# sdfgeoff/stereo_depth_estimation

Measured on AMD Instinct MI355X. Metric: stereo pairs/s training @320x240 bf16, 1/2/4/8 MI355X; EPE vs ref, higher is better.
Workload: dtype bf16

## Files before the change

stereo_depth_estimation_amd/csrc/conv_halo.hip:

```cpp
#include "common.h"
#include "halo_util.h"

namespace {

constexpr int CK = 32;
#ifndef WG_EXP
#define WG_EXP 0
#endif
typedef float f32x16 __attribute__((ext_vector_type(16)));

struct HaloSrc {
    const __bf16* p0;
    const __bf16* p1;
    const float *sc0, *sh0, *sc1, *sh1;
    int c0, c1, x0, x1;
    int ctot;
};
static inline HaloSrc make_halo_src(const sd_src& s) {
    HaloSrc h;
    h.p0 = (const __bf16*)s.ptr[0];
    h.p1 = (const __bf16*)s.ptr[1];
    h.sc0 = s.scale[0];
    h.sh0 = s.shift[0];
    h.sc1 = s.scale[1];
    h.sh1 = s.shift[1];
    h.c0 = s.chans[0];
    h.c1 = s.chans[1];
    h.x0 = s.xform[0];
    h.x1 = s.xform[1];
    h.ctot = s.chans[0] + s.chans[1];
    return h;
}

__device__ __forceinline__ uint4 bnrelu8(uint4 raw, const float* sc, const float* sh) {
    float v[8];
    const unsigned w[4] = {raw.x, raw.y, raw.z, raw.w};
#pragma unroll
    for (int i = 0; i < 4; ++i) {
        v[2 * i] = __uint_as_float(w[i] << 16);
        v[2 * i + 1] = __uint_as_float(w[i] & 0xffff0000u);
    }
    xform8(v, sc, sh, 0);
// ... 86 lines not shown
    int th, tw, tiles_x;
    int tiles, nsp;
    int nblk, gper;
    int hw, nhalo;
    const __bf16* wp;
    int N, kpad;
    int wsplit;
    const float* osc;
    const float* osh;
    int epi;
    __bf16* out0;
    __bf16* out1;
    int n_split;
    float* stats;
    int xcd;
    int prio;
    unsigned long long* dbg;
    const __bf16* by;
    const float *bsc, *bsh, *bmu, *bis;
    int ksplit, gblk, cps;
    int npix;
    float* part;
};

#ifndef HC_ST_AUX
#define HC_ST_AUX 2
#endif
#ifndef HC_WDMA
#define HC_WDMA 1
#endif
#ifndef HC_VR
#define HC_VR 1
#endif
__device__ __forceinline__ void stats_add(float* own, const uint4 v, const bool live) {
    const unsigned wv[4] = {live ? v.x : 0u, live ? v.y : 0u, live ? v.z : 0u, live ? v.w : 0u};
#pragma unroll
    for (int q = 0; q < 4; ++q) {
        const f32x2 x = {__uint_as_float(wv[q] << 16), __uint_as_float(wv[q] & 0xffff0000u)};
        f32x2 sm = {own[4 * q], own[4 * q + 1]}, sq = {own[4 * q + 2], own[4 * q + 3]};
        sm += x;
        sq = __builtin_elementwise_fma(x, x, sq);
        own[4 * q] = sm.x;
        own[4 * q + 1] = sm.y;
        own[4 * q + 2] = sq.x;
        own[4 * q + 3] = sq.y;
    }
}
template <bool B> struct BoolC { static constexpr bool v = B; };
constexpr int PERSIST_BLOCKS = 256;
constexpr int SBN_MAX = 1024;
constexpr int HMAX = 384;
__host__ __device__ constexpr int halo_px_cap(int RT, int CK) { return RT == 4 ? 640 : (RT == 3 && CK == 16 ? 512 : 384); }
__host__ __device__ constexpr int halo_ld(int CK) { return CK == 8 ? 8 : CK + 8; }
__host__ __device__ constexpr int wrow_ld(int CK) { return CK == 8 ? 88 : 9 * CK + 8; }
__device__ __forceinline__ int wswz(int row) { return ((row >> 2) & 1) * 2; }

template <int PPX>
__device__ __forceinline__ int ld_pixel(int item) { return (item / (8 * PPX)) * 8 + (item & 7); }
template <int PPX>
__device__ __forceinline__ int ld_piece(int item) { return (item >> 3) % PPX; }

template <int NT, int RT, int CK, bool STATS, bool WCONST, int IT, bool BNS, bool OAFF, bool RAW>
__device__ __forceinline__ void halo_conv_body(const HFwdArgs& p) {
    static_assert(!(OAFF && (STATS || BNS)), "the affine epilogue stores eval-mode outputs (no statistics)");
    constexpr int BN = 32 * NT;
    constexpr int PPX = CK / 8;
    constexpr bool M16 = CK == 32 && IT == 1 && !BNS;
    constexpr int HX_LD = halo_ld(CK), W_LD = M16 ? 9 * CK : wrow_ld(CK);
    constexpr int HPX = IT == 2 ? 384 : halo_px_cap(RT, CK);
    constexpr int HP = (HPX * PPX + 255) / 256;
    constexpr int WPIECES = BN * 9 * PPX;
    constexpr int W_PER_THREAD = (WPIECES + 255) / 256;
    static_assert(!M16 || (HP * 256 == HPX * PPX && HPX % 16 == 0), "M16: the loader pieces tile the halo exactly");
    constexpr int HALO_ITEM = M16 ? HPX * CK : HP * 256 / PPX * HX_LD;
    constexpr int HALO_ELEMS = IT * HALO_ITEM, W_ELEMS = BN * W_LD, BUF = HALO_ELEMS + W_ELEMS;
    static_assert(IT == 1 || (IT == 2 && HP * IT <= 16), "item masks fit 16 bits");
    constexpr int KS = (9 * CK + 15) / 16;
    __shared__ __attribute__((aligned(16))) __bf16 smem[2 * BUF];
    constexpr int SCR_PX = M16 ? 16 : 32;
    __shared__ __attribute__((aligned(16))) __bf16 scr[4 * SCR_PX * BN];

    const int tid = threadIdx.x, lane = tid & 63;
    const bool is_loader = (tid >> 6) >= 4;
    const int wid = (tid >> 6) & 3;
    const int bid = p.xcd ? (blockIdx.x & 7) * (gridDim.x >> 3) + (blockIdx.x >> 3) : blockIdx.x;
    const int ks = bid / p.gblk, bb = bid - ks * p.gblk;
    const int nb = bb % p.nblk, slot = bb / p.nblk;
    const int n0 = nb * BN;
    const int nc0 = (p.a.c0 + CK - 1) / CK;
    const int ncp = nc0 + (p.a.c1 + CK - 1) / CK;
    const int nch_v = p.wsplit ? 2 * ncp : ncp;
    const int c_lo = ks * p.cps;
    const int nchunks = (c_lo + p.cps < nch_v ? c_lo + p.cps : nch_v) - c_lo;
    const int wct = p.wsplit ? 2 * p.a.ctot : p.a.ctot;
    const int mvalid = p.th * p.tw;
    const int my_items = slot < p.nsp ? (p.nsp - 1 - slot) / p.gper + 1 : 0;
    const int total = (my_items + IT - 1) / IT * nchunks;
#ifndef HC_LS_N32
#define HC_LS_N32 2
#endif
    constexpr int LS = NT == 1 && CK == 8 ? 4 : (NT == 1 && CK == 32 ? HC_LS_N32 : 2);
    const int padded = (total + LS - 1) / LS * LS;

    __shared__ __attribute__((aligned(16))) float sbn[2 * SBN_MAX + 2 * CK];
    __shared__ __attribute__((aligned(16))) float oaff[OAFF ? 2 * BN : 4];
    auto fill_tables = [&]() __attribute__((always_inline)) {
        if constexpr (OAFF) {
            for (int c = tid; c < 2 * BN; c += 512) {
                const int ch = n0 + (c < BN ? c : c - BN);
                oaff[c] = ch < p.N ? (c < BN ? p.osc : p.osh)[ch] : 0.f;
            }
        }
        for (int c = tid; c < p.a.ctot; c += 512) {
            const bool first = c < p.a.c0;
            const int cl = first ? c : c - p.a.c0;
            const bool bn = (first ? p.a.x0 : p.a.x1) == SD_BNRELU;
            sbn[c] = bn ? (first ? p.a.sc0 : p.a.sc1)[cl] : 1.f;
            sbn[SBN_MAX + c] = bn ? (first ? p.a.sh0 : p.a.sh1)[cl] : 0.f;
        }
    };
    float* const redf = sbn;
    static_assert(4 * BN * 2 <= 2 * SBN_MAX, "redf fits in sbn");

    if (p.prio != 0 && (__builtin_amdgcn_readfirstlane(threadIdx.x) >= 256) == (p.prio == 2))
        __builtin_amdgcn_s_setprio(1);
    if (is_loader) {
        const int ltid = wid * 64 + lane;
        constexpr unsigned OOB = 0x80000000u;
        const int hw_img = p.H * p.W;
        const int lpiece = ld_piece<PPX>(ltid);
        unsigned pgeo[HP];
#pragma unroll
        for (int i = 0; i < HP; ++i) {
            const int px = ld_pixel<PPX>(ltid + i * 256);
            const int hy = px / p.hw;
            pgeo[i] = px < p.nhalo ? ((unsigned)hy << 16) | (unsigned)(px - hy * p.hw) : 0xffffffffu;
        }
        int hpx[IT][HP];
        const __bf16* ib0[IT];
        const __bf16* ib1[IT];
        int ld_pass = 0, ld_cc = 0;
        auto geometry = [&]() __attribute__((always_inline)) {
#pragma unroll
            for (int u = 0; u < IT; ++u) {
                const int itm = ld_pass * IT + u;
                const bool live = itm < my_items;
                const int sp = slot + (live ? itm : 0) * p.gper;
                const int b = sp / p.tiles, tl = sp - b * p.tiles;
                const int ty = tl / p.tiles_x;
                const int h0 = ty * p.th - 1, w0 = (tl - ty * p.tiles_x) * p.tw - 1;
                ib0[u] = p.a.p0 + (size_t)b * hw_img * p.a.c0;
                ib1[u] = p.a.c1 ? p.a.p1 + (size_t)b * hw_img * p.a.c1 : p.a.p0;
#pragma unroll
                for (int i = 0; i < HP; ++i) {
                    const int h = h0 + (int)(pgeo[i] >> 16), w = w0 + (int)(pgeo[i] & 0xffffu);
                    const bool in = live & (pgeo[i] != 0xffffffffu) & (h >= 0) & (w >= 0) & (h < p.H) & (w < p.W);
                    hpx[u][i] = in ? h * p.W + w : -1;
                }
            }
        };
        const __amdgpu_buffer_rsrc_t wrs =
            __builtin_amdgcn_make_buffer_rsrc((void*)p.wp, (short)0, p.N * p.kpad * 2, 0x00020000);
        constexpr bool WDMA = HC_WDMA && M16 && IT == 1 && (!WCONST || RAW);
        unsigned woff[W_PER_THREAD];
#pragma unroll
        for (int i = 0; i < W_PER_THREAD; ++i) {
            const int item = ltid + i * 256;
            const int co = item / (9 * PPX), r = item - co * (9 * PPX), tap = r / PPX, sp = r - tap * PPX;
// ... 60 lines not shown
        };
        auto load_w = [&]() __attribute__((always_inline)) { load_w_into(wr); };
        auto dma_w = [&](int buf) __attribute__((always_inline)) {
            const int wv = c_lo + w_cc;
            const bool lo = wv >= ncp;
            const int wc = lo ? wv - ncp : wv;
            const bool s1 = wc >= nc0;
            const int cl = (s1 ? wc - nc0 : wc) * CK;
            if (++w_cc == nchunks) w_cc = 0;
            const unsigned soff = __builtin_amdgcn_readfirstlane(((s1 ? p.a.c0 : 0) + cl + (lo ? p.a.ctot : 0)) * 2);
            const unsigned m0b = __builtin_amdgcn_readfirstlane(lds_w0 + (unsigned)(buf * BUF * 2));
#pragma unroll
            for (int j = 0; j < WDI; ++j) {
                if (NWI % 4 != 0 && wid_u * WDI + j >= NWI) break;
                unsigned keep;
                asm volatile(
                    "s_mov_b32 %0, m0\n\t"
                    "s_mov_b32 m0, %2\n\t"
                    "s_nop 0\n\t"
                    "buffer_load_dwordx4 %1, %3, %4 offen lds\n\t"
                    "s_mov_b32 m0, %0"
                    : "=&s"(keep)
                    : "v"(wdoff[j]), "s"(m0b + (unsigned)j * 1024u), "s"(wrs), "s"(soff)
                    : "memory");
            }
        };
        if constexpr (RAW) {
            static_assert(M16 && PPX == 4 && HPX % 64 == 0 && WDMA, "RAW: the M16 piece-major halo, weights by DMA");
            constexpr int HI = HPX / 64;
            unsigned hg[HI];
#pragma unroll
            for (int i = 0; i < HI; ++i) {
                const int px = i * 64 + lane;
                const int hy = px / p.hw;
                hg[i] = px < p.nhalo ? ((unsigned)hy << 16) | (unsigned)(px - hy * p.hw) : 0xffffffffu;
            }
            int hp[HI];
            const __bf16 *rb0 = p.a.p0, *rb1 = p.a.p0;
            int r_pass = 0, r_cc = 0;
            auto rgeo = [&]() __attribute__((always_inline)) {
                const bool live = r_pass < my_items;
                const int sp = slot + (live ? r_pass : 0) * p.gper;
                const int b = sp / p.tiles, tl = sp - b * p.tiles;
                const int ty = tl / p.tiles_x;
                const int h0 = ty * p.th - 1, w0 = (tl - ty * p.tiles_x) * p.tw - 1;
                rb0 = p.a.p0 + (size_t)b * hw_img * p.a.c0;
                rb1 = p.a.c1 ? p.a.p1 + (size_t)b * hw_img * p.a.c1 : p.a.p0;
#pragma unroll
                for (int i = 0; i < HI; ++i) {
                    const int h = h0 + (int)(hg[i] >> 16), w = w0 + (int)(hg[i] & 0xffffu);
                    const bool in = live & (hg[i] != 0xffffffffu) & (h >= 0) & (w >= 0) & (h < p.H) & (w < p.W);
                    hp[i] = in ? h * p.W + w : -1;
                }
            };
            rgeo();
            const unsigned lds_h0 = (unsigned)(uintptr_t)smem + (unsigned)(wid_u * HPX * 16);
            fill_tables();
            __syncthreads();
            if constexpr (WCONST) {
                dma_w(0);
                dma_w(1);
            }
            for (int g = 0; g < padded; ++g) {
                if (g < total) {
                    const int hv = c_lo + r_cc;
                    const int hc = hv >= ncp ? hv - ncp : hv;
                    const bool s1 = hc >= nc0;
// ... 94 lines not shown
#pragma unroll
            for (int u = 0; u < IT; ++u)
#pragma unroll
            for (int i = 0; i < HP; ++i) {
                const int item = ltid + i * 256;
                uint4 v = q.hr[u][i];
                const bool ok = (q.m >> (u * HP + i)) & 1u;
                if (q.bn && !(WG_EXP & 2048)) {
                    v = bnrelu_pk(v, s0, s1, h0, h1);
                    v = ok ? v : make_uint4(0, 0, 0, 0);
                }
                const int hoff = M16 ? ld_piece<PPX>(item) * HPX * 8 + ld_pixel<PPX>(item) * 8
                                     : ld_pixel<PPX>(item) * HX_LD + ld_piece<PPX>(item) * 8;
                *reinterpret_cast<uint4*>(hx + u * HALO_ITEM + hoff) = v;
            }
            if constexpr (!WCONST && !WDMA) if (!(WG_EXP & 131072)) store_w(buf);
        };
        constexpr std::integral_constant<int, 0> S0{};
        constexpr std::integral_constant<int, 1> S1{};
        constexpr std::integral_constant<int, 2> S2{};
        constexpr std::integral_constant<int, 3> S3{};
        constexpr bool DG = (WG_EXP & 1024) != 0;
        unsigned long long t_st = 0, t_ld = 0, t_br = 0, t0 = 0, t_all = DG ? __builtin_amdgcn_s_memtime() : 0;
        auto stamp = [&](unsigned long long& acc_) __attribute__((always_inline)) {
            if (DG) {
                asm volatile("s_waitcnt lgkmcnt(0)" ::: "memory");
                const unsigned long long t1 = __builtin_amdgcn_s_memtime();
                acc_ += t1 - t0;
                t0 = t1;
            } else if (WG_EXP & 8192) {
                asm volatile("s_waitcnt lgkmcnt(0)" ::: "memory");
            }
        };
        auto iter = [&](auto U) __attribute__((always_inline)) {
            if (DG) t0 = __builtin_amdgcn_s_memtime();
            if (!(WG_EXP & 65536)) store(U, decltype(U)::value & 1);
            stamp(t_st);
            if constexpr (WDMA) {
                __builtin_amdgcn_sched_barrier(0);
                dma_w(decltype(U)::value & 1);
                __builtin_amdgcn_sched_barrier(0);
            } else if constexpr (!WCONST) {
                if (!(WG_EXP & 65536)) load_w();
            }
            if (!(WG_EXP & 65536)) load(U);
            stamp(t_ld);
            if constexpr (WDMA && !(WG_EXP & 4194304)) {
                __builtin_amdgcn_sched_barrier(0);
                asm volatile("s_waitcnt vmcnt(%0)" ::"i"(IT * HP) : "memory");
            }
            __syncthreads();
            stamp(t_br);
        };
        uint4 wr2[WCONST ? W_PER_THREAD : 1];
        if (total > 0) {
            geometry();
            if constexpr (WCONST) {
                load_w();
                if (nchunks > 1) load_w_into(wr2);
                __builtin_amdgcn_sched_barrier(0);
            }
            load(S0);
            __builtin_amdgcn_sched_barrier(0);
            if constexpr (LS == 4) {
                load(S1);
                __builtin_amdgcn_sched_barrier(0);
                load(S2);
                __builtin_amdgcn_sched_barrier(0);
            }
            if constexpr (!WCONST && !WDMA) load_w();
            __builtin_amdgcn_sched_barrier(0);
            if constexpr (LS == 4) load(S3);
            else load(S1);
        }
        fill_tables();
        __syncthreads();
        if (total > 0) {
            if constexpr (WCONST) {
                store_w(0);
                if (nchunks > 1) store_w_from(1, wr2);
                else store_w(1);
            }
            for (int gi = 0; gi < total; gi += LS) {
                iter(S0);
                iter(S1);
                if constexpr (LS == 4) {
                    iter(S2);
                    iter(S3);
                }
            }
        }
        if (DG && p.dbg && lane == 0) {
            unsigned long long* d = p.dbg + ((size_t)blockIdx.x * 8 + 4 + wid) * 4;
            d[0] = t_st;
            d[1] = t_ld;
            d[2] = t_br;
            d[3] = __builtin_amdgcn_s_memtime() - t_all;
        }
        __syncthreads();
        return;
    }

    fill_tables();
    __syncthreads();
    static_assert(!(STATS && BNS), "one kind of stats rows");
    constexpr int NOWN = STATS || BNS ? 16 : 1;
    float own[NOWN];
#pragma unroll
    for (int j = 0; j < NOWN; ++j) own[j] = 0.f;
    constexpr int PPP = NT * 4;
    constexpr bool VR32 = HC_VR && !M16 && NT == 1 && RT == 4 && CK == 32 && IT == 1;
    auto tile_T = [&](int i) { return M16 || VR32 ? wid * RT + i : wid + 4 * i; };
    constexpr bool VR = HC_VR && M16 && NT == 1 && RT == 4;
    int abase[RT];
#pragma unroll
    for (int i = 0; i < RT; ++i) {
        const int m = tile_T(i) * 32 + (lane & 31);
        const int hm = m / p.tw, wm = m - hm * p.tw;
        abase[i] = m < mvalid ? hm * p.hw + wm : 0;
    }
    int abase16[M16 ? 2 * RT : 1];
    if constexpr (M16) {
#pragma unroll
        for (int i = 0; i < 2 * RT; ++i) {
            const int m = tile_T(i >> 1) * 32 + (i & 1) * 16 + (lane & 15);
            const int hm = m / p.tw, wm = m - hm * p.tw;
            abase16[i] = (lane >> 4) * HPX * 8 + (m < mvalid ? hm * p.hw + wm : 0) * 8;
        }
    }
    f32x16 acc[M16 ? 1 : IT][M16 ? 1 : RT][M16 ? 1 : NT];
    f32x4 acc4[M16 ? 2 * RT : 1][M16 ? 2 * NT : 1];
    constexpr int EPR = 64 / PPP;
    constexpr int ER = 32 / EPR;
    auto swz = [](int j, int px) { return NT == 2 ? j ^ (px & 7) : j ^ ((px >> 1) & 3); };
    unsigned erel[(RT * ER + 1) / 2];
#pragma unroll
    for (int k = 0; k < (RT * ER + 1) / 2; ++k) erel[k] = 0xffffffffu;
#pragma unroll
    for (int i = 0; i < RT; ++i)
#pragma unroll
        for (int r = 0; r < ER; ++r) {
            const int m = tile_T(i) * 32 + r * EPR + lane / PPP;
            const int hm = m / p.tw, wm = m - hm * p.tw;
            const unsigned v = m < mvalid ? (unsigned)((hm << 9) | wm) : 0xffffu;
            const int k = i * ER + r;
            erel[k / 2] = (erel[k / 2] & ~(0xffffu << (16 * (k & 1)))) | (v << (16 * (k & 1)));
        }
    constexpr bool EFAST = M16 && !(NT == 2 && RT == 3);
    constexpr int NEO = EFAST ? RT * ER : 1;
    int eoff[NEO];
#pragma unroll
    for (int k = 0; k < NEO; ++k) {
        const int m = tile_T(k / ER) * 32 + (k % ER) * EPR + lane / PPP;
        const int hm = m / p.tw, wm = m - hm * p.tw;
        eoff[k] = m < mvalid ? hm * p.W + wm : -1;
    }
    __bf16* const scw = scr + wid * SCR_PX * BN;
    constexpr int NBK = BNS ? 8 : 1, NYQ = BNS ? RT * ER : 1;
    BnsK bk[NBK / 2 > 0 ? NBK / 2 : 1];
    uint4 yq[NYQ];
    if constexpr (BNS) {
        const int c = n0 + (lane % PPP) * 8;
#pragma unroll
        for (int q = 0; q < 4; ++q) {
            float v[4][2];
#pragma unroll
            for (int h = 0; h < 2; ++h) {
                const int ch = c + 2 * q + h;
                const bool cin = ch < p.N;
                v[0][h] = cin ? p.bsc[ch] : 0.f;
                v[1][h] = cin ? p.bsh[ch] : 0.f;
                v[2][h] = cin ? p.bis[ch] : 0.f;
                v[3][h] = cin ? -p.bmu[ch] * p.bis[ch] : 0.f;
            }
            bk[q].sc = f32x2{v[0][0], v[0][1]};
            bk[q].sh = f32x2{v[1][0], v[1][1]};
            bk[q].is = f32x2{v[2][0], v[2][1]};
            bk[q].nmi = f32x2{v[3][0], v[3][1]};
        }
    }
    auto prefetch_y = [&](int itm) __attribute__((always_inline)) {
        const int sp = slot + itm * p.gper;
        const int b = sp / p.tiles, tl = sp - b * p.tiles;
        const int ty = tl / p.tiles_x;
        const int h0 = ty * p.th, w0 = (tl - ty * p.tiles_x) * p.tw;
        const int hw_img = p.H * p.W;
        const __amdgpu_buffer_rsrc_t ry = __builtin_amdgcn_make_buffer_rsrc(
            (void*)(p.by + (size_t)b * hw_img * p.N), (short)0, hw_img * p.N * 2, 0x00020000);
#pragma unroll
        for (int k = 0; k < RT * ER; ++k) {
            const unsigned rel = (erel[k / 2] >> (16 * (k & 1))) & 0xffffu;
            const int h = h0 + (int)(rel >> 9), w = w0 + (int)(rel & 511u);
            const int c = n0 + (lane % PPP) * 8;
            const bool in = (rel != 0xffffu) & (h < p.H) & (w < p.W) & (c < p.N);
            const unsigned off = in ? (unsigned)((h * p.W + w) * p.N + c) * 2u : 0x80000000u;
            const auto v = __builtin_amdgcn_raw_buffer_load_b128(ry, off, 0, 0);
            yq[k] = make_uint4(v[0], v[1], v[2], v[3]);
        }
    };

    constexpr bool DG = (WG_EXP & 1024) != 0;
    unsigned long long t_cp = 0, t_ep = 0, t_br = 0, t0 = 0, t_all = DG ? __builtin_amdgcn_s_memtime() : 0;
    int cc = 0, pass = 0;
    for (int gi = 0; gi < total; ++gi) {
        if (DG) t0 = __builtin_amdgcn_s_memtime();
        if (WG_EXP & 16384) {
            asm volatile("" ::: "memory");
            __builtin_amdgcn_sched_barrier(0);
        }
        __syncthreads();
        if (DG) {
            const unsigned long long t1 = __builtin_amdgcn_s_memtime();
            t_br += t1 - t0;
            t0 = t1;
        }
        if (WG_EXP & 16384) {
            asm volatile("" ::: "memory");
            __builtin_amdgcn_sched_barrier(0);
        }
        if (cc == 0) {
            if constexpr (M16) {
#pragma unroll
                for (int i = 0; i < 2 * RT; ++i)
#pragma unroll
                    for (int t = 0; t < 2 * NT; ++t) acc4[i][t] = f32x4{0.f, 0.f, 0.f, 0.f};
            } else {
#pragma unroll
            for (int u = 0; u < IT; ++u)
#pragma unroll
            for (int i = 0; i < RT; ++i)
#pragma unroll
                for (int t = 0; t < NT; ++t)
#pragma unroll
                    for (int r = 0; r < 16; ++r) acc[u][i][t][r] = 0.f;
            }
        }
        if constexpr (BNS) {
            if (cc == nchunks - 1) prefetch_y(pass);
        }
        const __bf16* hx = smem + (gi & 1) * BUF;
        const __bf16* wl = hx + HALO_ELEMS;
#ifndef HC_PF
#define HC_PF 1
#endif
        constexpr int PF = HC_PF;
        bf16x8 af[PF + 1][IT][RT], bfr[PF + 1][NT];
        auto read_frags = [&](int step) {
// ... 120 lines not shown
                __builtin_amdgcn_sched_barrier(0);
#pragma unroll
                for (int kh = 0; kh < 3; ++kh) {
                    const int r = hr - kh;
                    if (r < 0 || r >= R) continue;
                    acc[0][r][0] = __builtin_amdgcn_mfma_f32_32x32x16_bf16(av[kh][ch], xv[st % (PV + 1)], acc[0][r][0], 0,
                                                                           0, 0);
                }
                __builtin_amdgcn_sched_barrier(0);
            }
        } else if (!(WG_EXP & 8)) {
#pragma unroll
        for (int step = 0; step < PF; ++step) read_frags(step);
#pragma unroll
        for (int step = 0; step < KS; ++step) {
            if (step + PF < KS) read_frags(step + PF);
            __builtin_amdgcn_sched_barrier(0);
            const int sl = step % (PF + 1);
#pragma unroll
            for (int u = 0; u < IT; ++u)
#pragma unroll
            for (int i = 0; i < RT; ++i)
#pragma unroll
                for (int t = 0; t < NT; ++t)
                    acc[u][i][t] = __builtin_amdgcn_mfma_f32_32x32x16_bf16(bfr[sl][t], af[sl][u][i], acc[u][i][t], 0, 0, 0);
            __builtin_amdgcn_sched_barrier(0);
        }
        }

        if (DG) {
            const unsigned long long t1 = __builtin_amdgcn_s_memtime();
            t_cp += t1 - t0;
            t0 = t1;
        }
        if (WG_EXP & 16384) {
            asm volatile("" ::: "memory");
            __builtin_amdgcn_sched_barrier(0);
        }
        if (++cc == nchunks) {
#pragma unroll
          for (int u = 0; u < IT; ++u) {
            const int item = pass * IT + u;
            if (IT > 1 && item >= my_items) break;
            const int sp = slot + item * p.gper;
            const int b = sp / p.tiles, tl = sp - b * p.tiles;
            const int ty = tl / p.tiles_x;
            const int h0 = ty * p.th, w0 = (tl - ty * p.tiles_x) * p.tw;
            const int hw_img = p.H * p.W;
            if constexpr (!STATS && !BNS) {
                if (p.part) {
                    float* const pk = p.part + ((size_t)ks * p.npix + (size_t)b * hw_img) * p.N;
                    auto put = [&](int m, int c, float a0, float a1, float a2, float a3) __attribute__((always_inline)) {
                        const int hm = m / p.tw, wm = m - hm * p.tw;
                        if ((m < mvalid) & (h0 + hm < p.H) & (w0 + wm < p.W) & (n0 + c < p.N))
                            *reinterpret_cast<float4*>(pk + ((size_t)(h0 + hm) * p.W + w0 + wm) * p.N + n0 + c) =
                                make_float4(a0, a1, a2, a3);
                    };
                    if constexpr (M16) {
#pragma unroll
                        for (int i2 = 0; i2 < 2 * RT; ++i2)
#pragma unroll
                            for (int t = 0; t < 2 * NT; ++t)
                                put(tile_T(i2 >> 1) * 32 + (i2 & 1) * 16 + (lane & 15), t * 16 + 4 * (lane >> 4),
                                    acc4[i2][t][0], acc4[i2][t][1], acc4[i2][t][2], acc4[i2][t][3]);
                    } else {
#pragma unroll
// ... 157 lines not shown
                    const unsigned rel = (erel[(i * ER + r) / 2] >> (16 * ((i * ER + r) & 1))) & 0xffffu;
                    const int h = h0 + (int)(rel >> 9), w = w0 + (int)(rel & 511u);
                    const bool live = (rel != 0xffffu) & (h < p.H) & (w < p.W);
                    const bool in = live & !(WG_EXP & 4096);
                    const int pix = h * p.W + w, c = n0 + j * 8;
                    if constexpr (BNS) {
                        bns_add(own, v, yq[i * ER + r], live, bk);
                    }
                    if constexpr (STATS) {
                        stats_add(own, v, live);
                    }
                    __attribute__((ext_vector_type(4))) unsigned data = {v.x, v.y, v.z, v.w};
                    if (!split) {
                        const unsigned off = (in & (c < p.N)) ? (unsigned)(pix * p.N + c) * 2u : 0x80000000u;
                        __builtin_amdgcn_raw_buffer_store_b128(data, rs0, off, 0, HC_ST_AUX);
                    } else {
                        const unsigned o0 = (in & (c < ns)) ? (unsigned)(pix * ns + c) * 2u : 0x80000000u;
                        const unsigned o1 = (in & (c >= ns) & (c < p.N)) ? (unsigned)(pix * (p.N - ns) + c - ns) * 2u
                                                                       : 0x80000000u;
                        __builtin_amdgcn_raw_buffer_store_b128(data, rs0, o0, 0, HC_ST_AUX);
                        __builtin_amdgcn_raw_buffer_store_b128(data, rs1, o1, 0, HC_ST_AUX);
                    }
                }
              }
            }
            }
          }
            cc = 0;
            ++pass;
            if (DG) {
                const unsigned long long t1 = __builtin_amdgcn_s_memtime();
                t_ep += t1 - t0;
                t0 = t1;
            }
        }
    }
    for (int e = total; e < padded; ++e) __syncthreads();
    if (DG && p.dbg && lane == 0) {
        unsigned long long* d = p.dbg + ((size_t)blockIdx.x * 8 + wid) * 4;
        d[0] = t_cp;
        d[1] = t_ep;
        d[2] = t_br;
        d[3] = __builtin_amdgcn_s_memtime() - t_all;
    }

    if constexpr (STATS || BNS) {
#pragma unroll
        for (int k = 0; k < NOWN; ++k) {
#pragma unroll
            for (int o = PPP; o < 64; o <<= 1) own[k] += __shfl_xor(own[k], o);
        }
        if (lane < PPP) {
#pragma unroll
            for (int k = 0; k < NOWN; ++k)
                redf[(wid * BN + lane * 8 + k / 2) * 2 + (k & 1)] =
                    own[(k & ~3) | ((k & 1) << 1) | ((k >> 1) & 1)];
        }
    }
    __syncthreads();
    if ((STATS || BNS) && tid < BN && n0 + tid < p.N) {
        float s = 0.f, ss = 0.f;
#pragma unroll
        for (int w = 0; w < 4; ++w) {
            s += redf[(w * BN + tid) * 2];
            ss += redf[(w * BN + tid) * 2 + 1];
        }
        reinterpret_cast<float2*>(p.stats)[(size_t)slot * p.N + n0 + tid] = make_float2(s, ss);
    }
}

template <int NT, int RT, int CK, bool STATS, bool WCONST, int IT, bool BNS, bool OAFF = false, bool RAW = false>
__global__ __launch_bounds__(512) void k_halo_conv(const HFwdArgs p) {
    halo_conv_body<NT, RT, CK, STATS, WCONST, IT, BNS, OAFF, RAW>(p);
}

struct HWgArgs {
    const __bf16* dy;
    HaloSrc x;
    int H, W, th, tw, hw, nhalo, tiles_x, tiles_y, ntiles, tiles_per_split;
    int M, N;
    float* slab;
    int xcd;
    unsigned long long* dbg;
    const __bf16* bda;
    const __bf16* by;
    const float *bsc, *bsh, *bmu, *bis, *bcoef;
    int ncc;
};

constexpr int XW_LD = CK + 16;
__device__ __forceinline__ int wg_pixel(int item) { return (item >> 5) * 8 + ((item >> 3) & 1) * 4 + ((item >> 1) & 3); }
__device__ __forceinline__ int wg_piece(int item) { return (item & 1) + ((item >> 4) & 1) * 2; }
constexpr int HP_PER_THREAD = HMAX * (CK / 8) / 256;
constexpr int WG_MAXPX = 256;



template <int COUT, bool BNB, bool X8 = false>
__global__ __launch_bounds__(256, 2) void k_halo_wgrad(const HWgArgs p) {
    constexpr int DY_LD = COUT + 16;
// ... 311 lines not shown
        for (int h = 0; h < 2; ++h) {
            const int m = ks * 16 + pk + 8 * h;
            const int hm = m / p.tw;
            const int px = m < mvalid ? hm * HP + (m - hm * p.tw) : 0;
            xoff[ks][h] = (unsigned)(px * XLD + ch16) * 2u;
        }
    const unsigned aoff = (unsigned)(pk * DLD + ch16) * 2u;
    switch (__builtin_amdgcn_readfirstlane(wid)) {
    case 0: ws_mfma32_tiles<HP, DLD, XLD, DY_E, BUF, 0>(p, smem, lane, cc, mb, split, ntile, xoff, aoff); break;
    case 1: ws_mfma32_tiles<HP, DLD, XLD, DY_E, BUF, 1>(p, smem, lane, cc, mb, split, ntile, xoff, aoff); break;
    case 2: ws_mfma32_tiles<HP, DLD, XLD, DY_E, BUF, 2>(p, smem, lane, cc, mb, split, ntile, xoff, aoff); break;
    default: ws_mfma32_tiles<HP, DLD, XLD, DY_E, BUF, 3>(p, smem, lane, cc, mb, split, ntile, xoff, aoff); break;
    }
}

template <int COUT, int CIB, int HP, int HR, bool BNB, bool SPAN, bool MF32 = false>
__global__ __launch_bounds__(512, 2 * ws_blocks_per_cu(COUT, CIB)) void k_halo_wgrad_ws(const HWgArgs p) {
    constexpr int KS = WS_TPX / 32;
    constexpr int NCI = CIB / 16, NCO = 4 / NCI, RM = COUT / 16 / NCO;
    constexpr int DPP = COUT / 8, XPP = CIB / 8;
    constexpr int PAD = MF32 ? 32 : 16;
    constexpr int DLD = COUT + PAD, XLD = CIB + PAD;
    constexpr int DYP = WS_TPX * DPP / 256;
    constexpr int HXP = (HP * HR * XPP + 255) / 256;
    constexpr int DY_E = WS_TPX * DLD, BUF = DY_E + HXP * (256 / XPP) * XLD;
    static_assert(RM >= 1 && NCI * NCO == 4, "wave grid");
    static_assert(!MF32 || (COUT == 64 && CIB == 64 && !SPAN), "MF32: 64 x 64 blocks");
    static_assert(2 * BUF * 2 <= 160 * 1024, "LDS");
    __shared__ __attribute__((aligned(16))) __bf16 smem[2 * BUF];

    const int tid = threadIdx.x, lane = tid & 63;
    const bool is_loader = tid >= 256;
    const int wid = (tid >> 6) & 3;
    int cc = blockIdx.x, zb = blockIdx.z, split = blockIdx.y;
    if (p.xcd) {
        const int G = gridDim.x * gridDim.y * gridDim.z;
        const int L = blockIdx.x + gridDim.x * (blockIdx.y + gridDim.y * blockIdx.z);
        const int lg = (L & 7) * (G >> 3) + (L >> 3);
        cc = lg % gridDim.x;
        const int r = lg / gridDim.x;
        zb = r % gridDim.z;
        split = r / gridDim.z;
    }
    const int mb = zb * COUT;
    const int t_begin = split * p.tiles_per_split;
    const int ntile = max(0, min(p.ntiles, t_begin + p.tiles_per_split) - t_begin);
    const int mvalid = p.th * p.tw;

    if (is_loader) {
        constexpr int prio = (COUT == 128 && !BNB) ? 0 : WS_PRIO;
        if (prio) __builtin_amdgcn_s_setprio(prio);
        const int ltid = tid - 256;
        const int dpiece = ltid % DPP, dpix0 = ltid / DPP, xpiece = ltid % XPP, xpix0 = ltid / XPP;
        unsigned dyrc[(DYP + 1) / 2], hgeo[(HXP + 1) / 2];
#pragma unroll
        for (int i = 0; i < DYP; i += 2) {
            unsigned e[2];
#pragma unroll
            for (int h = 0; h < 2; ++h) {
                const int m = dpix0 + (256 / DPP) * (i + h);
                const int hm = m / p.tw;
                e[h] = (i + h < DYP && m < mvalid) ? (unsigned)(hm << 8 | (m - hm * p.tw)) : 0xffffu;
            }
            dyrc[i / 2] = e[0] | e[1] << 16;
        }
#pragma unroll
        for (int i = 0; i < HXP; i += 2) {
            unsigned e[2];
#pragma unroll
            for (int h = 0; h < 2; ++h) {
                const int px = xpix0 + (256 / XPP) * (i + h);
                const int hy = px / HP, hx = px - hy * HP;
                e[h] = (i + h < HXP && hy < p.th + 2 && hx < p.hw) ? (unsigned)(hy << 8 | hx) : 0xffffu;
            }
            hgeo[i / 2] = e[0] | e[1] << 16;
        }
        const HaloCol hc = halo_col(p.x, cc * CIB + xpiece * 8, p.slab);
        const bool bsrc1 = cc * CIB >= p.x.c0;
        const __bf16* xsrc = bsrc1 ? p.x.p1 : p.x.p0;
        const int xC = SPAN ? hc.C : (bsrc1 ? p.x.c1 : p.x.c0);
        const bool lsrc1 = SPAN && cc * CIB + xpiece * 8 >= p.x.c0;
        int dpo[DYP], xpo[HXP];
#pragma unroll
        for (int i = 0; i < DYP; ++i) {
            const unsigned rc = (dyrc[i / 2] >> (16 * (i & 1))) & 0xffffu;
            dpo[i] = ((int)(rc >> 8) * p.W + (int)(rc & 0xff)) * p.M + mb + dpiece * 8;
        }
#pragma unroll
        for (int i = 0; i < HXP; ++i) {
            const unsigned gg = (hgeo[i / 2] >> (16 * (i & 1))) & 0xffffu;
            xpo[i] = (((int)(gg >> 8) - 1) * p.W + (int)(gg & 0xff) - 1) * xC + hc.c;
        }
        constexpr bool DYDMA = WS_DYDMA && !BNB && !SPAN && (DLD * 2) % 16 == 0;
        constexpr int RS = DLD / 8;
        constexpr int NDI = (WS_TPX * RS + 63) / 64;
        constexpr int DDI = DYDMA ? (NDI + 3) / 4 : 1;
        const int lw = __builtin_amdgcn_readfirstlane(wid);
        int ddo[DDI];
        unsigned ddrc[DDI];
        if constexpr (DYDMA) {
#pragma unroll
            for (int j = 0; j < DDI; ++j) {
                const int k = lw * DDI + j, sl = k * 64 + lane;
                const int m = sl / RS, pc = sl - m * RS;
                const int hm = m / p.tw, wm = m - hm * p.tw;
                const bool ok = k < NDI && pc < DPP && m < mvalid && m < WS_TPX;
                ddo[j] = ok ? (hm * p.W + wm) * p.M + mb + pc * 8 : -1;
                ddrc[j] = ok ? (unsigned)(hm << 8 | wm) : 0xffffu;
            }
        }
        const unsigned lds_dy0 = (unsigned)(uintptr_t)smem + (unsigned)(lw * DDI) * 1024u;
        constexpr int NK = BNB ? 8 : 1;
        float ksc[NK], ksh[NK], kB[NK], kC[NK];
        if constexpr (BNB) {
            const int c = mb + dpiece * 8;
#pragma unroll
            for (int j = 0; j < 8; ++j) {
                const float k1 = p.bcoef[3 * (c + j) + 1], k2 = p.bcoef[3 * (c + j) + 2];
                const float is = p.bis[c + j], sc = p.bsc[c + j], sh = p.bsh[c + j];
                ksc[j] = sc;
                ksh[j] = sh;
                kB[j] = -is * k2;
                kC[j] = is * k2 * sh + sc * (p.bmu[c + j] * is * k2 - k1);
            }
        }
        constexpr int DYY = BNB ? DYP : 1;
        constexpr unsigned OOB = 0x80000000u;
        struct TSet {
            uint4 d[DYP], x[HXP];
            unsigned xm;
            uint4 y[DYY];
            int dbase;
            int img;
            bool wr;
        };
        TSet sa, sb;
        auto load = [&](TSet& q, int tile) __attribute__((always_inline)) {
            if (WG_EXP & 256) return;
// ... 86 lines not shown
                    (WG_EXP & 2048) ? q.x[i] : halo_finish_pk(hc, (q.xm >> i) & 1u, q.x[i]);
        };
        constexpr bool DG = (WG_EXP & 1024) != 0;
        unsigned long long t_st = 0, t_ld = 0, t_br = 0, t0 = 0, t1 = 0, t_all = DG ? __builtin_amdgcn_s_memtime() : 0;
        auto dma_dy = [&](int buf, int tile) __attribute__((always_inline)) {
            const int tx = tile % p.tiles_x;
            const int rest = tile / p.tiles_x;
            const int ty = rest % p.tiles_y, b = rest / p.tiles_y;
            const int h0 = ty * p.th, w0 = tx * p.tw;
            const int nimg = p.H * p.W;
            const __amdgpu_buffer_rsrc_t rdy = __builtin_amdgcn_make_buffer_rsrc(
                (void*)(p.dy + (size_t)b * nimg * p.M), (short)0, nimg * p.M * 2, 0x00020000);
            int rhi = p.H - h0, chi = p.W - w0;
            if (tile >= t_begin + ntile) rhi = 0;
            const int dbase = (h0 * p.W + w0) * p.M;
            const unsigned m0b = __builtin_amdgcn_readfirstlane(lds_dy0 + (unsigned)(buf * BUF * 2));
#pragma unroll
            for (int j = 0; j < DDI; ++j) {
                if (NDI % 4 != 0 && lw * DDI + j >= NDI) break;
                const bool ok = (ddo[j] >= 0) & ((int)(ddrc[j] >> 8) < rhi) & ((int)(ddrc[j] & 0xffu) < chi);
                const unsigned off = ok ? (unsigned)(dbase + ddo[j]) * 2u : OOB;
                unsigned keep;
                asm volatile(
                    "s_mov_b32 %0, m0\n\t"
                    "s_mov_b32 m0, %2\n\t"
                    "s_nop 0\n\t"
                    "buffer_load_dwordx4 %1, %3, 0 offen lds\n\t"
                    "s_mov_b32 m0, %0"
                    : "=&s"(keep)
                    : "v"(off), "s"(m0b + (unsigned)j * 1024u), "s"(rdy)
                    : "memory");
            }
        };
        auto iter = [&](TSet& q, int buf, int tile) __attribute__((always_inline)) {
            if (DG) t0 = __builtin_amdgcn_s_memtime();
            store(q, buf);
            if (DG) { asm volatile("s_waitcnt lgkmcnt(0)" ::: "memory"); t1 = __builtin_amdgcn_s_memtime(); t_st += t1 - t0; }
            if constexpr (DYDMA) {
                __builtin_amdgcn_sched_barrier(0);
                dma_dy(buf, tile - 2);
                __builtin_amdgcn_sched_barrier(0);
            }
            load(q, tile);
            if (DG) { t0 = t1; t1 = __builtin_amdgcn_s_memtime(); t_ld += t1 - t0; t0 = t1; }
            if constexpr (DYDMA) {
                __builtin_amdgcn_sched_barrier(0);
                asm volatile("s_waitcnt vmcnt(%0)" ::"i"(HXP) : "memory");
            }
            __syncthreads();
            if (DG) t_br += __builtin_amdgcn_s_memtime() - t0;
        };
        load(sa, t_begin);
        __builtin_amdgcn_sched_barrier(0);
        load(sb, t_begin + 1);
        for (int i = 0; i < ntile; i += 2) {
            iter(sa, 0, t_begin + i + 2);
            iter(sb, 1, t_begin + i + 3);
        }
        if (DG && p.dbg && lane == 0) {
            unsigned long long* d = p.dbg + ((size_t)(blockIdx.x + gridDim.x * (blockIdx.y + gridDim.y * blockIdx.z)) * 8 + 4 + wid) * 4;
            d[0] = t_st;
            d[1] = t_ld;
            d[2] = t_br;
            d[3] = __builtin_amdgcn_s_memtime() - t_all;
        }
        return;
    }

    if constexpr (MF32) {
        ws_mfma32<HP, DLD, XLD, DY_E, BUF>(p, smem, lane, wid, cc, mb, split, ntile, mvalid);
        return;
    }
    const int g = lane >> 4, q = (lane & 15) >> 2, pp = lane & 3;
    const int pc = 16 * (g >> 1) + 4 * (g & 1) + q;
    const int ci0 = 16 * (wid % NCI), co0 = (wid / NCI) * (COUT / NCO);
    unsigned xoff[KS][2];
#pragma unroll
    for (int ks = 0; ks < KS; ++ks)
#pragma unroll
        for (int h = 0; h < 2; ++h) {
            const int m = ks * 32 + pc + 8 * h;
            const int hm = m / p.tw;
            const int px = m < mvalid ? hm * HP + (m - hm * p.tw) : 0;
            xoff[ks][h] = (unsigned)(px * XLD + ci0 + 4 * pp) * 2u;
        }
    f32x4 acc[9][RM];
#pragma unroll
    for (int t = 0; t < 9; ++t)
#pragma unroll
        for (int i = 0; i < RM; ++i) acc[t][i] = f32x4{0.f, 0.f, 0.f, 0.f};

    constexpr int NSTEP = KS * 9;
    bf16x8 bring[WS_PD + 1];
    bf16x8 aring[2][RM];
    const char* lds = reinterpret_cast<const char*>(smem);
    constexpr bool DG = (WG_EXP & 1024) != 0;
    unsigned long long t_cp = 0, t_br = 0, t0 = 0, t_all = DG ? __builtin_amdgcn_s_memtime() : 0;
    for (int it = 0; it < ntile; ++it) {
        if (DG) t0 = __builtin_amdgcn_s_memtime();
        __syncthreads();
        if (DG) {
            const unsigned long long t1 = __builtin_amdgcn_s_memtime();
            t_br += t1 - t0;
            t0 = t1;
        }
        const unsigned bufb = (unsigned)((it & 1) * BUF * 2);
        unsigned abase = bufb + (unsigned)(pc * DLD + co0 + 4 * pp) * 2u;
        asm volatile("" : "+v"(abase));
        unsigned xb[KS][2];
#pragma unroll
        for (int ks = 0; ks < KS; ++ks)
#pragma unroll
            for (int h = 0; h < 2; ++h) {
                xb[ks][h] = xoff[ks][h] + bufb + (unsigned)(DY_E * 2);
                asm volatile("" : "+v"(xb[ks][h]));
            }
        auto issue = [&](int j) __attribute__((always_inline)) {
            const int ks = j / 9, tap = j - ks * 9;
            if (tap == 0) {
#pragma unroll
                for (int i = 0; i < RM; ++i) {
                    const __bf16* a0 = reinterpret_cast<const __bf16*>(lds + abase) + ks * 32 * DLD + i * 16;
                    aring[ks & 1][i] = tr_pair(a0, a0 + 8 * DLD);
                }
            }
            const int toff = ((tap / 3) * HP + tap % 3) * XLD;
            bring[j % (WS_PD + 1)] = tr_pair(reinterpret_cast<const __bf16*>(lds + xb[ks][0]) + toff,
                                             reinterpret_cast<const __bf16*>(lds + xb[ks][1]) + toff);
        };
        if (!(WG_EXP & 64)) {
#pragma unroll
            for (int j = 0; j < WS_PD; ++j) issue(j);
#pragma unroll
            for (int j = 0; j < NSTEP; ++j) {
                if (j + WS_PD < NSTEP) issue(j + WS_PD);
                __builtin_amdgcn_sched_barrier(0);
                const int ks = j / 9, tap = j - ks * 9;
#pragma unroll
                for (int i = 0; i < RM; ++i)
                    acc[tap][i] = __builtin_amdgcn_mfma_f32_16x16x32_bf16(aring[ks & 1][i], bring[j % (WS_PD + 1)],
                                                                         acc[tap][i], 0, 0, 0);
                __builtin_amdgcn_sched_barrier(0);
            }
        }
        if (DG) t_cp += __builtin_amdgcn_s_memtime() - t0;
    }
    if (ntile & 1) __syncthreads();
    if (DG && p.dbg && lane == 0) {
        unsigned long long* d = p.dbg + ((size_t)(blockIdx.x + gridDim.x * (blockIdx.y + gridDim.y * blockIdx.z)) * 8 + wid) * 4;
        d[0] = t_cp;
        d[1] = 0;
        d[2] = t_br;
        d[3] = __builtin_amdgcn_s_memtime() - t_all;
    }
    float* slab = p.slab + (size_t)split * p.M * p.N;
    const int ci = cc * CIB + ci0 + (lane & 15);
#pragma unroll
    for (int tap = 0; tap < 9; ++tap)
#pragma unroll
        for (int i = 0; i < RM; ++i)
#pragma unroll
            for (int r = 0; r < 4; ++r) {
                const int co = mb + co0 + i * 16 + 4 * (lane >> 4) + r;
                slab[(size_t)co * p.N + tap * p.x.ctot + ci] = acc[tap][i][r];
            }
}

}

static unsigned long long* g_wg_dbg = nullptr;
extern "C" int sd_debug_buffer(void* p) {
    g_wg_dbg = (unsigned long long*)p;
    return 0;
}
unsigned long long* sd_debug_ptr() { return g_wg_dbg; }

bool sd_halo_fwd_shape(int N) { return N == 32 || N % 64 == 0; }
bool sd_halo_fwd_ok(const sd_src& a, int N, int epi) {
    return a.taps == 9 && !a.pool && sd_halo_fwd_shape(N) && epi != SD_EPI_PIXSHUF &&
           a.chans[0] + a.chans[1] <= SBN_MAX;
}

static bool halo_xcd_enabled() {
    static const bool on = [] {
        const char* e = getenv("SD_HALO_XCD");
        return !(e && atoi(e) == 0);
    }();
    return on;
}

static bool wg_x8(int ctot) {
    const char* e = getenv("SD_WG_X8");
    if (e && *e && atoi(e) == 0) return false;
    return ctot > 0 && ctot <= 8;
}

static bool halo_raw_enabled() {
    const char* e = getenv("SD_HALO_RAW");
// ... 419 lines not shown
        for (int tw = W < 8 ? W : 8; tw <= (W < l[0] - 2 ? W : l[0] - 2); ++tw) {
            if (tw != W && tw != 32 && W % tw) continue;
            for (int th = 1; th <= H && th * tw <= WS_TPX && th + 2 <= l[1]; ++th) {
                const double tiles = (double)cdiv(H, th) * cdiv(W, tw);
                const double cost = tiles * (WS_TPX + 1.0 * slots);
                if (cost < best_cost) {
                    best_cost = cost;
                    best = {th, tw, l[0], l[1]};
                }
            }
        }
    }
    return best;
}

static bool ws_mf32_enabled() {
    const char* e = getenv("SD_WS_MF32");
    return e && atoi(e) == 1;
}

static bool ws_co128_enabled() {
    const char* e = getenv("SD_WS_CO128");
    return !(e && atoi(e) == 0);
}
static WsCfg wgrad_ws_launch(int M, int N, int c0, bool bnb) {
    WsCfg c = wgrad_ws(M, N, c0);
    if (!bnb && c.cout == 64 && c.cib && !c.span && M % 128 == 0 && (N / 9) % 32 == 0 && c0 % 32 == 0 &&
        ws_co128_enabled())
        c = WsCfg{128, 32};
    return c;
}

int sd_halo_wgrad_splits(int batch, int H, int W, int M, int N) {
    const WsCfg ws = wgrad_ws(M, N);
    HTile t = wgrad_tile(H, W);
    if (ws.cib) {
        const WsTile w = wgrad_tile_ws(H, W);
        t = {w.th, w.tw, 4, 32};
    }
    const int nblk = ws.cib ? (N / 9 / ws.cib) * (M / ws.cout) : cdiv(N / 9, CK) * (M == 32 ? 1 : M / 64);
    const int nt = cdiv(W, t.tw) * cdiv(H, t.th) * batch;
    static const int blocks = [] {
        const char* e = getenv("SD_WG_BLOCKS");
        return e && atoi(e) > 0 ? atoi(e) : 512;
    }();
    int splits = cdiv(ws.cib ? PERSIST_BLOCKS * ws_blocks_per_cu(ws.cout, ws.cib) : blocks, nblk);
    if (splits > nt) splits = nt;
    return splits < 1 ? 1 : splits;
}

const char* sd_halo_wgrad_name(int M, int N, int c0, int H, int W, bool bnb) {
    static thread_local char buf[64];
    const WsCfg ws = wgrad_ws_launch(M, N, c0, bnb);
    if (!ws.cib)
        return M == 32 ? (bnb ? (wg_x8(c0) ? "k_halo_wgrad<32, true, true>" : "k_halo_wgrad<32, true>")
                              : "k_halo_wgrad<32, false>")
                       : "k_halo_wgrad<64, false>";
    const WsTile t = wgrad_tile_ws(H, W);
    const bool mf32 = ws.cout == 64 && ws.cib == 64 && ws_mf32_enabled();
    snprintf(buf, sizeof(buf), "k_halo_wgrad_ws<%d, %d, %d, %d, %s, %s%s>", ws.cout, ws.cib, t.hp, t.hr, bnb ? "true" : "false",
             ws.span ? "true" : "false", mf32 ? ", true" : "");
    return buf;
}

template <int COUT, int CIB, bool BNB, bool SPAN = false, bool MF32 = false>
static void launch_wgrad_ws(int hp, dim3 grid, hipStream_t st, const HWgArgs& p) {
    if (hp == 34)
        hipLaunchKernelGGL((k_halo_wgrad_ws<COUT, CIB, 34, 6, BNB, SPAN, MF32>), grid, dim3(512), 0, st, p);
    else
        hipLaunchKernelGGL((k_halo_wgrad_ws<COUT, CIB, 22, 8, BNB, SPAN, MF32>), grid, dim3(512), 0, st, p);
}
template <bool BNB>
static void launch_wgrad_ws(const WsCfg& ws, int hp, dim3 grid, hipStream_t st, const HWgArgs& p) {
    if (!BNB && ws.cout == 128) launch_wgrad_ws<128, 32, false>(hp, grid, st, p);
    else if (ws.cout == 64 && ws.cib == 64 && ws_mf32_enabled()) launch_wgrad_ws<64, 64, BNB, false, true>(hp, grid, st, p);
    else if (ws.cout == 64 && ws.cib == 64) launch_wgrad_ws<64, 64, BNB>(hp, grid, st, p);
    else if (ws.cout == 64) launch_wgrad_ws<64, 32, BNB>(hp, grid, st, p);
    else if (ws.cib == 64 && ws.span) launch_wgrad_ws<32, 64, BNB, true>(hp, grid, st, p);
    else if (ws.cib == 64) launch_wgrad_ws<32, 64, BNB>(hp, grid, st, p);
    else launch_wgrad_ws<32, 32, BNB>(hp, grid, st, p);
}

int sd_halo_wgrad_bnbwd_blocks(const sd_src& a, const sd_src& b, int M, int N) {
    if (!sd_halo_wgrad_ok(a, b, M)) return 0;
    const WsCfg ws = wgrad_ws(M, N, b.chans[0]);
    if (ws.cib) return (N / 9) / ws.cib;
    return M == 32 && !a.ptr[0] ? cdiv(b.chans[0] + b.chans[1], CK) : 0;
}
// ... 65 lines not shown
```

Measured before the change: 7690.

## Replace integer divisions by float reciprocal multiply and fix wgrad split count

Replaces per-pixel integer divisions by tile width and halo width with a float reciprocal multiply (enabled by default via HC_FDIV), cutting the cost of integer division in index setup. Adjusts the wgrad split computation to use COUT=128 when the launch path does, so the grid sizing matches the kernel actually launched, and fixes the kernel name lookup to use N/9. It also adds phase timestamp instrumentation that is compiled only in debug builds. The float division trick is exact only for small operands.

```diff
diff --git a/stereo_depth_estimation_amd/csrc/conv_halo.hip b/stereo_depth_estimation_amd/csrc/conv_halo.hip
--- a/stereo_depth_estimation_amd/csrc/conv_halo.hip
+++ b/stereo_depth_estimation_amd/csrc/conv_halo.hip
@@ -8,6 +8,19 @@
 #define WG_EXP 0
 #endif
 typedef float f32x16 __attribute__((ext_vector_type(16)));
+
+constexpr bool DG_BUILD = (WG_EXP & 1024) != 0;
+constexpr int DBG_PHASE0 = 2048 * 32, DBG_PHASE_BLOCKS = 4096;
+__device__ __forceinline__ unsigned long long phase_clock() {
+    if constexpr (!DG_BUILD) return 0;
+    __builtin_amdgcn_sched_barrier(0);
+    const unsigned long long t = __builtin_amdgcn_s_memrealtime();
+    __builtin_amdgcn_sched_barrier(0);
+    return t;
+}
+__device__ __forceinline__ void phase_retire(float v) {
+    if (DG_BUILD) asm volatile("" ::"s"(__builtin_amdgcn_readfirstlane(__float_as_int(v))));
+}
 
 struct HaloSrc {
     const __bf16* p0;
@@ -160,6 +173,12 @@
 #ifndef HC_VR
 #define HC_VR 1
 #endif
+#ifndef HC_FDIV
+#define HC_FDIV 1
+#endif
+__device__ __forceinline__ int small_div(int m, int d, float rd) {
+    return HC_FDIV ? (int)(((float)m + 0.5f) * rd) : m / d;
+}
 __device__ __forceinline__ void stats_add(float* own, const uint4 v, const bool live) {
     const unsigned wv[4] = {live ? v.x : 0u, live ? v.y : 0u, live ? v.z : 0u, live ? v.w : 0u};
 #pragma unroll
@@ -211,6 +230,7 @@
     const int tid = threadIdx.x, lane = tid & 63;
     const bool is_loader = (tid >> 6) >= 4;
     const int wid = (tid >> 6) & 3;
+    const unsigned long long ph_entry = phase_clock();
     const int bid = p.xcd ? (blockIdx.x & 7) * (gridDim.x >> 3) + (blockIdx.x >> 3) : blockIdx.x;
     const int ks = bid / p.gblk, bb = bid - ks * p.gblk;
     const int nb = bb % p.nblk, slot = bb / p.nblk;
@@ -222,6 +242,7 @@
     const int nchunks = (c_lo + p.cps < nch_v ? c_lo + p.cps : nch_v) - c_lo;
     const int wct = p.wsplit ? 2 * p.a.ctot : p.a.ctot;
     const int mvalid = p.th * p.tw;
+    const float rtw = 1.f / (float)p.tw, rhw = 1.f / (float)p.hw;
     const int my_items = slot < p.nsp ? (p.nsp - 1 - slot) / p.gper + 1 : 0;
     const int total = (my_items + IT - 1) / IT * nchunks;
 #ifndef HC_LS_N32
@@ -261,7 +282,7 @@
 #pragma unroll
         for (int i = 0; i < HP; ++i) {
             const int px = ld_pixel<PPX>(ltid + i * 256);
-            const int hy = px / p.hw;
+            const int hy = small_div(px, p.hw, rhw);
             pgeo[i] = px < p.nhalo ? ((unsigned)hy << 16) | (unsigned)(px - hy * p.hw) : 0xffffffffu;
         }
         int hpx[IT][HP];
@@ -388,7 +409,7 @@
 #pragma unroll
             for (int i = 0; i < HI; ++i) {
                 const int px = i * 64 + lane;
-                const int hy = px / p.hw;
+                const int hy = small_div(px, p.hw, rhw);
                 hg[i] = px < p.nhalo ? ((unsigned)hy << 16) | (unsigned)(px - hy * p.hw) : 0xffffffffu;
             }
             int hp[HI];
@@ -549,10 +570,12 @@
                 asm volatile("s_waitcnt lgkmcnt(0)" ::: "memory");
             }
         };
+        unsigned long long lp_issued = 0, lp_halo = 0, lp_dma = 0;
         auto iter = [&](auto U) __attribute__((always_inline)) {
             if (DG) t0 = __builtin_amdgcn_s_memtime();
             if (!(WG_EXP & 65536)) store(U, decltype(U)::value & 1);
             stamp(t_st);
+            if (DG && lp_halo == 0) lp_halo = phase_clock();
             if constexpr (WDMA) {
                 __builtin_amdgcn_sched_barrier(0);
                 dma_w(decltype(U)::value & 1);
@@ -566,6 +589,7 @@
                 __builtin_amdgcn_sched_barrier(0);
                 asm volatile("s_waitcnt vmcnt(%0)" ::"i"(IT * HP) : "memory");
             }
+            if (DG && lp_dma == 0) lp_dma = phase_clock();
             __syncthreads();
             stamp(t_br);
         };
@@ -589,6 +613,7 @@
             __builtin_amdgcn_sched_barrier(0);
             if constexpr (LS == 4) load(S3);
             else load(S1);
+            lp_issued = phase_clock();
         }
         fill_tables();
         __syncthreads();
@@ -613,6 +638,12 @@
             d[1] = t_ld;
             d[2] = t_br;
             d[3] = __builtin_amdgcn_s_memtime() - t_all;
+            if (wid == 0 && blockIdx.x < DBG_PHASE_BLOCKS) {
+                unsigned long long* e = p.dbg + DBG_PHASE0 + (size_t)blockIdx.x * 16 + 8;
+                e[0] = lp_issued;
+                e[1] = lp_halo;
+                e[2] = lp_dma;
+            }
         }
         __syncthreads();
         return;
@@ -633,7 +664,7 @@
 #pragma unroll
     for (int i = 0; i < RT; ++i) {
         const int m = tile_T(i) * 32 + (lane & 31);
-        const int hm = m / p.tw, wm = m - hm * p.tw;
+        const int hm = small_div(m, p.tw, rtw), wm = m - hm * p.tw;
         abase[i] = m < mvalid ? hm * p.hw + wm : 0;
     }
     int abase16[M16 ? 2 * RT : 1];
@@ -641,7 +672,7 @@
 #pragma unroll
         for (int i = 0; i < 2 * RT; ++i) {
             const int m = tile_T(i >> 1) * 32 + (i & 1) * 16 + (lane & 15);
-            const int hm = m / p.tw, wm = m - hm * p.tw;
+            const int hm = small_div(m, p.tw, rtw), wm = m - hm * p.tw;
             abase16[i] = (lane >> 4) * HPX * 8 + (m < mvalid ? hm * p.hw + wm : 0) * 8;
         }
     }
@@ -658,7 +689,7 @@
 #pragma unroll
         for (int r = 0; r < ER; ++r) {
             const int m = tile_T(i) * 32 + r * EPR + lane / PPP;
-            const int hm = m / p.tw, wm = m - hm * p.tw;
+            const int hm = small_div(m, p.tw, rtw), wm = m - hm * p.tw;
             const unsigned v = m < mvalid ? (unsigned)((hm << 9) | wm) : 0xffffu;
             const int k = i * ER + r;
             erel[k / 2] = (erel[k / 2] & ~(0xffffu << (16 * (k & 1)))) | (v << (16 * (k & 1)));
@@ -669,7 +700,7 @@
 #pragma unroll
     for (int k = 0; k < NEO; ++k) {
         const int m = tile_T(k / ER) * 32 + (k % ER) * EPR + lane / PPP;
-        const int hm = m / p.tw, wm = m - hm * p.tw;
+        const int hm = small_div(m, p.tw, rtw), wm = m - hm * p.tw;
         eoff[k] = m < mvalid ? hm * p.W + wm : -1;
     }
     __bf16* const scw = scr + wid * SCR_PX * BN;
@@ -718,8 +749,10 @@
 
     constexpr bool DG = (WG_EXP & 1024) != 0;
     unsigned long long t_cp = 0, t_ep = 0, t_br = 0, t0 = 0, t_all = DG ? __builtin_amdgcn_s_memtime() : 0;
+    unsigned long long ph_arrive = 0, ph_first = 0, ph_retire = 0, ph_store = 0;
     int cc = 0, pass = 0;
     for (int gi = 0; gi < total; ++gi) {
+        if (DG && gi == 0) ph_arrive = phase_clock();
         if (DG) t0 = __builtin_amdgcn_s_memtime();
         if (WG_EXP & 16384) {
             asm volatile("" ::: "memory");
@@ -730,6 +763,7 @@
             const unsigned long long t1 = __builtin_amdgcn_s_memtime();
             t_br += t1 - t0;
             t0 = t1;
+            if (gi == 0) ph_first = phase_clock();
         }
         if (WG_EXP & 16384) {
             asm volatile("" ::: "memory");
@@ -916,6 +950,22 @@
             const unsigned long long t1 = __builtin_amdgcn_s_memtime();
             t_cp += t1 - t0;
             t0 = t1;
+            if (gi == total - 1) {
+                if constexpr (M16) {
+#pragma unroll
+                    for (int i = 0; i < 2 * RT; ++i)
+#pragma unroll
+                        for (int t = 0; t < 2 * NT; ++t) phase_retire(acc4[i][t][0]);
+                } else {
+#pragma unroll
+                    for (int u = 0; u < IT; ++u)
+#pragma unroll
+                        for (int i = 0; i < RT; ++i)
+#pragma unroll
+                            for (int t = 0; t < NT; ++t) phase_retire(acc[u][i][t][0]);
+                }
+                ph_retire = phase_clock();
+            }
         }
         if (WG_EXP & 16384) {
             asm volatile("" ::: "memory");
@@ -1139,6 +1189,7 @@
                 const unsigned long long t1 = __builtin_amdgcn_s_memtime();
                 t_ep += t1 - t0;
                 t0 = t1;
+                if (gi == total - 1) ph_store = phase_clock();
             }
         }
     }
@@ -1173,6 +1224,16 @@
             ss += redf[(w * BN + tid) * 2 + 1];
         }
         reinterpret_cast<float2*>(p.stats)[(size_t)slot * p.N + n0 + tid] = make_float2(s, ss);
+    }
+    if (DG && p.dbg && tid == 0 && blockIdx.x < DBG_PHASE_BLOCKS) {
+        unsigned long long* d = p.dbg + DBG_PHASE0 + (size_t)blockIdx.x * 16;
+        d[0] = ph_entry;
+        d[1] = ph_first;
+        d[2] = ph_retire;
+        d[3] = ph_store;
+        d[4] = phase_clock();
+        d[5] = (unsigned long long)my_items;
+        d[6] = ph_arrive;
     }
 }
 
@@ -1550,6 +1611,7 @@
     const int tid = threadIdx.x, lane = tid & 63;
     const bool is_loader = tid >= 256;
     const int wid = (tid >> 6) & 3;
+    const unsigned long long ph_entry = phase_clock();
     int cc = blockIdx.x, zb = blockIdx.z, split = blockIdx.y;
     if (p.xcd) {
         const int G = gridDim.x * gridDim.y * gridDim.z;
@@ -1564,6 +1626,7 @@
     const int t_begin = split * p.tiles_per_split;
     const int ntile = max(0, min(p.ntiles, t_begin + p.tiles_per_split) - t_begin);
     const int mvalid = p.th * p.tw;
+    const float rtw = 1.f / (float)p.tw;
 
     if (is_loader) {
         constexpr int prio = (COUT == 128 && !BNB) ? 0 : WS_PRIO;
@@ -1577,7 +1640,7 @@
 #pragma unroll
             for (int h = 0; h < 2; ++h) {
                 const int m = dpix0 + (256 / DPP) * (i + h);
-                const int hm = m / p.tw;
+                const int hm = small_div(m, p.tw, rtw);
                 e[h] = (i + h < DYP && m < mvalid) ? (unsigned)(hm << 8 | (m - hm * p.tw)) : 0xffffu;
             }
             dyrc[i / 2] = e[0] | e[1] << 16;
@@ -1621,7 +1684,7 @@
             for (int j = 0; j < DDI; ++j) {
                 const int k = lw * DDI + j, sl = k * 64 + lane;
                 const int m = sl / RS, pc = sl - m * RS;
-                const int hm = m / p.tw, wm = m - hm * p.tw;
+                const int hm = small_div(m, p.tw, rtw), wm = m - hm * p.tw;
                 const bool ok = k < NDI && pc < DPP && m < mvalid && m < WS_TPX;
                 ddo[j] = ok ? (hm * p.W + wm) * p.M + mb + pc * 8 : -1;
                 ddrc[j] = ok ? (unsigned)(hm << 8 | wm) : 0xffffu;
@@ -1774,10 +1837,12 @@
                     : "memory");
             }
         };
+        unsigned long long lp_issued = 0, lp_halo = 0, lp_dma = 0;
         auto iter = [&](TSet& q, int buf, int tile) __attribute__((always_inline)) {
             if (DG) t0 = __builtin_amdgcn_s_memtime();
             store(q, buf);
             if (DG) { asm volatile("s_waitcnt lgkmcnt(0)" ::: "memory"); t1 = __builtin_amdgcn_s_memtime(); t_st += t1 - t0; }
+            if (DG && lp_halo == 0) lp_halo = phase_clock();
             if constexpr (DYDMA) {
                 __builtin_amdgcn_sched_barrier(0);
                 dma_dy(buf, tile - 2);
@@ -1789,12 +1854,14 @@
                 __builtin_amdgcn_sched_barrier(0);
                 asm volatile("s_waitcnt vmcnt(%0)" ::"i"(HXP) : "memory");
             }
+            if (DG && lp_dma == 0) lp_dma = phase_clock();
             __syncthreads();
             if (DG) t_br += __builtin_amdgcn_s_memtime() - t0;
         };
         load(sa, t_begin);
         __builtin_amdgcn_sched_barrier(0);
         load(sb, t_begin + 1);
+        lp_issued = phase_clock();
         for (int i = 0; i < ntile; i += 2) {
             iter(sa, 0, t_begin + i + 2);
             iter(sb, 1, t_begin + i + 3);
@@ -1805,6 +1872,13 @@
             d[1] = t_ld;
             d[2] = t_br;
             d[3] = __builtin_amdgcn_s_memtime() - t_all;
+            const unsigned lin = blockIdx.x + gridDim.x * (blockIdx.y + gridDim.y * blockIdx.z);
+            if (wid == 0 && lin < (unsigned)DBG_PHASE_BLOCKS) {
+                unsigned long long* e = p.dbg + DBG_PHASE0 + (size_t)lin * 16 + 8;
+                e[0] = lp_issued;
+                e[1] = lp_halo;
+                e[2] = lp_dma;
+            }
         }
         return;
     }
@@ -1822,7 +1896,7 @@
 #pragma unroll
         for (int h = 0; h < 2; ++h) {
             const int m = ks * 32 + pc + 8 * h;
-            const int hm = m / p.tw;
+            const int hm = small_div(m, p.tw, rtw);
             const int px = m < mvalid ? hm * HP + (m - hm * p.tw) : 0;
             xoff[ks][h] = (unsigned)(px * XLD + ci0 + 4 * pp) * 2u;
         }
@@ -1838,13 +1912,16 @@
     const char* lds = reinterpret_cast<const char*>(smem);
     constexpr bool DG = (WG_EXP & 1024) != 0;
     unsigned long long t_cp = 0, t_br = 0, t0 = 0, t_all = DG ? __builtin_amdgcn_s_memtime() : 0;
+    unsigned long long ph_arrive = 0, ph_first = 0, ph_retire = 0;
     for (int it = 0; it < ntile; ++it) {
+        if (DG && it == 0) ph_arrive = phase_clock();
         if (DG) t0 = __builtin_amdgcn_s_memtime();
         __syncthreads();
         if (DG) {
             const unsigned long long t1 = __builtin_amdgcn_s_memtime();
             t_br += t1 - t0;
             t0 = t1;
+            if (it == 0) ph_first = phase_clock();
         }
         const unsigned bufb = (unsigned)((it & 1) * BUF * 2);
         unsigned abase = bufb + (unsigned)(pc * DLD + co0 + 4 * pp) * 2u;
@@ -1885,7 +1962,16 @@
                 __builtin_amdgcn_sched_barrier(0);
             }
         }
-        if (DG) t_cp += __builtin_amdgcn_s_memtime() - t0;
+        if (DG) {
+            t_cp += __builtin_amdgcn_s_memtime() - t0;
+            if (it == ntile - 1) {
+#pragma unroll
+                for (int t = 0; t < 9; ++t)
+#pragma unroll
+                    for (int i = 0; i < RM; ++i) phase_retire(acc[t][i][0]);
+                ph_retire = phase_clock();
+            }
+        }
     }
     if (ntile & 1) __syncthreads();
     if (DG && p.dbg && lane == 0) {
@@ -1906,6 +1992,16 @@
                 const int co = mb + co0 + i * 16 + 4 * (lane >> 4) + r;
                 slab[(size_t)co * p.N + tap * p.x.ctot + ci] = acc[tap][i][r];
             }
+    const unsigned lin = blockIdx.x + gridDim.x * (blockIdx.y + gridDim.y * blockIdx.z);
+    if (DG && p.dbg && tid == 0 && lin < (unsigned)DBG_PHASE_BLOCKS) {
+        unsigned long long* d = p.dbg + DBG_PHASE0 + (size_t)lin * 16;
+        d[0] = ph_entry;
+        d[1] = ph_first;
+        d[2] = ph_retire;
+        d[3] = d[4] = phase_clock();
+        d[5] = (unsigned long long)ntile;
+        d[6] = ph_arrive;
+    }
 }
 
 }
@@ -2391,7 +2487,8 @@
 }
 
 int sd_halo_wgrad_splits(int batch, int H, int W, int M, int N) {
-    const WsCfg ws = wgrad_ws(M, N);
+    WsCfg ws = wgrad_ws(M, N);
+    if (ws.cout == 64 && ws.cib == 32 && M % 128 == 0 && ws_co128_enabled()) ws.cout = 128;
     HTile t = wgrad_tile(H, W);
     if (ws.cib) {
         const WsTile w = wgrad_tile_ws(H, W);
@@ -2412,7 +2509,7 @@
     static thread_local char buf[64];
     const WsCfg ws = wgrad_ws_launch(M, N, c0, bnb);
     if (!ws.cib)
-        return M == 32 ? (bnb ? (wg_x8(c0) ? "k_halo_wgrad<32, true, true>" : "k_halo_wgrad<32, true>")
+        return M == 32 ? (bnb ? (wg_x8(N / 9) ? "k_halo_wgrad<32, true, true>" : "k_halo_wgrad<32, true>")
                               : "k_halo_wgrad<32, false>")
                        : "k_halo_wgrad<64, false>";
     const WsTile t = wgrad_tile_ws(H, W);
```

After: 7669. Within noise of the previous version (-0.3%).
